# Julian-Wyatt/AnoDDPM

Hardware: AMD Instinct MI355X
Metric: reverse-diffusion images/sec @256x256 T=1000 simplex (higher is better)
Workload: dtype f32; 1 GPU; 256x256 simplex(8 oct) T=1000 base128 attn16,8 batch4/GPU (BASELINE config 2); per_gpu_batch=4, global_batch=4, T=1000, parallelism=batch-sharded x1 (no data-path collective), output_finite=True

## Files before the change

anoddpm_amd/csrc/attention.hip:

```cpp
#include "common.h"

namespace {

typedef float f32x4 __attribute__((ext_vector_type(4)));

constexpr int AT_LMAX = 1024;
constexpr int AT_WAVES = 8;
constexpr int AT_NT = AT_WAVES * 64;

template <int CHQ>
__global__ __launch_bounds__(AT_NT) void attention_kernel(const anoddpm_attention_args a)
{
    constexpr int CH = CHQ * 16;
    constexpr int QP = CH + 4;
    constexpr int TPW = CHQ >= AT_WAVES ? CHQ / AT_WAVES : 1;
    __shared__ __attribute__((aligned(16))) float lds[16 * (AT_LMAX + 4) + 16 * QP];
    const int L = a.L, SP = L + 4;
    float *S = lds, *Qs = lds + 16 * (AT_LMAX + 4);
    const int tid = threadIdx.x, lane = tid & 63, wave = tid >> 6;
    const int l16 = lane & 15, kq = lane >> 4;
    const int row0 = blockIdx.x * 16, hd = blockIdx.y, b = blockIdx.z;
    const int C3 = 3 * a.heads * CH;
    const float *__restrict__ qkv = a.qkv + (int64_t)b * L * C3 + hd * 3 * CH;
    const int nkt = L >> 4;

    for (int idx = tid; idx < 16 * (CH / 4); idx += AT_NT) {
        const int r = idx / (CH / 4), c4 = idx - r * (CH / 4);
        *reinterpret_cast<f32x4 *>(Qs + r * QP + c4 * 4) = *reinterpret_cast<const f32x4 *>(qkv + (int64_t)(row0 + r) * C3 + c4 * 4);
    }
    constexpr bool DB = CHQ < 32;
    f32x4 kb[DB ? 2 : 1][CHQ];
    auto load_k = [&](f32x4 (&dst)[CHQ], int jt) {
        const float *kp = qkv + (int64_t)(jt * 16 + l16) * C3 + CH + kq * 4;
#pragma unroll
        for (int g = 0; g < CHQ; ++g) dst[g] = *reinterpret_cast<const f32x4 *>(kp + g * 16);
    };
    auto score_tile = [&](const f32x4 (&kk)[CHQ], int jt) {
        f32x4 acc = {0.f, 0.f, 0.f, 0.f};
#pragma unroll
        for (int g = 0; g < CHQ; ++g) {
            const f32x4 qa = *reinterpret_cast<const f32x4 *>(Qs + l16 * QP + g * 16 + kq * 4);
#pragma unroll
            for (int e = 0; e < 4; ++e) acc = __builtin_amdgcn_mfma_f32_16x16x4f32(qa[e], kk[g][e], acc, 0, 0, 0);
        }
#pragma unroll
        for (int r = 0; r < 4; ++r) S[(kq * 4 + r) * SP + jt * 16 + l16] = acc[r] * a.scale;
    };
    if (wave < nkt) load_k(kb[0], wave);
    __syncthreads();
    if constexpr (DB) {
        for (int jt = wave; jt < nkt; jt += 2 * AT_WAVES) {
            if (jt + AT_WAVES < nkt) load_k(kb[1], jt + AT_WAVES);
            score_tile(kb[0], jt);
            if (jt + AT_WAVES < nkt) {
                if (jt + 2 * AT_WAVES < nkt) load_k(kb[0], jt + 2 * AT_WAVES);
                score_tile(kb[1], jt + AT_WAVES);
            }
        }
    } else {
        for (int jt = wave; jt < nkt; jt += AT_WAVES) {
            if (jt != wave) load_k(kb[0], jt);
            score_tile(kb[0], jt);
        }
    }
    const int ct0 = wave * TPW;
    const bool pv_active = ct0 < CHQ;
    float vb[2][TPW][4];
    auto load_v = [&](float (&dst)[TPW][4], int kg) {
        const float *vp = qkv + (int64_t)(kg * 16 + kq * 4) * C3 + 2 * CH + ct0 * 16 + l16;
#pragma unroll
        for (int t = 0; t < TPW; ++t)
#pragma unroll
            for (int e = 0; e < 4; ++e) dst[t][e] = vp[(int64_t)e * C3 + t * 16];
    };
    if (pv_active) load_v(vb[0], 0);
    __syncthreads();

    {
        constexpr int TPR = AT_NT / 16;
        const int r = tid / TPR, sub = tid % TPR;
        float *srow = S + r * SP;
        float m = -INFINITY;
        for (int j = sub; j < L; j += TPR) m = fmaxf(m, srow[j]);
#pragma unroll
        for (int o = TPR / 2; o >= 1; o >>= 1) m = fmaxf(m, __shfl_xor(m, o, TPR));
        float sum = 0.f;
        for (int j = sub; j < L; j += TPR) {
            const float e = __expf(srow[j] - m);
            srow[j] = e;
            sum += e;
        }
#pragma unroll
        for (int o = TPR / 2; o >= 1; o >>= 1) sum += __shfl_xor(sum, o, TPR);
        const float inv = 1.0f / sum;
        float *prow = a.probs ? a.probs + (((int64_t)b * a.heads + hd) * L + row0 + r) * L : nullptr;
        for (int j = sub; j < L; j += TPR) {
            const float p = srow[j] * inv;
            srow[j] = p;
            if (prow) prow[j] = p;
        }
    }
    __syncthreads();

    if (!pv_active) return;
    f32x4 oacc[TPW];
#pragma unroll
    for (int t = 0; t < TPW; ++t) oacc[t] = f32x4{0.f, 0.f, 0.f, 0.f};
    auto pv_group = [&](const float (&vv)[TPW][4], int kg) {
        const f32x4 pa = *reinterpret_cast<const f32x4 *>(S + l16 * SP + kg * 16 + kq * 4);
#pragma unroll
        for (int e = 0; e < 4; ++e)
#pragma unroll
            for (int t = 0; t < TPW; ++t) oacc[t] = __builtin_amdgcn_mfma_f32_16x16x4f32(pa[e], vv[t][e], oacc[t], 0, 0, 0);
    };
    for (int kg = 0; kg < nkt; kg += 2) {
        if (kg + 1 < nkt) load_v(vb[1], kg + 1);
        pv_group(vb[0], kg);
        if (kg + 1 < nkt) {
            if (kg + 2 < nkt) load_v(vb[0], kg + 2);
            pv_group(vb[1], kg + 1);
        }
    }
    float *__restrict__ O = a.out + ((int64_t)b * L + row0 + kq * 4) * (a.heads * CH) + hd * CH + ct0 * 16 + l16;
#pragma unroll
    for (int t = 0; t < TPW; ++t)
#pragma unroll
        for (int r = 0; r < 4; ++r) O[(int64_t)r * (a.heads * CH) + t * 16] = oacc[t][r];
}

}

extern "C" int anoddpm_attention(const anoddpm_attention_args *a, void *stream)
{
    ANODDPM_REQUIRE(a && a->qkv && a->out, "attention: null pointer");
    ANODDPM_REQUIRE(a->B >= 1 && a->heads >= 1 && a->B <= 65535 && a->heads <= 65535, "attention: bad batch / head count");
    ANODDPM_REQUIRE(a->L >= 16 && a->L % 16 == 0 && a->L <= AT_LMAX, "attention: L must be a multiple of 16 in [16, 1024]");
    ANODDPM_REQUIRE(a->ch >= 16 && a->ch <= 512 && (a->ch & (a->ch - 1)) == 0, "attention: head width must be a power of two in [16, 512]");
    ANODDPM_REQUIRE(((uintptr_t)a->qkv & 15) == 0, "attention: qkv must be 16-byte aligned");
    const dim3 grid((unsigned)(a->L / 16), (unsigned)a->heads, (unsigned)a->B);
    hipStream_t s = anoddpm::as_stream(stream);
    switch (a->ch / 16) {
        case 1: hipLaunchKernelGGL((attention_kernel<1>), grid, dim3(AT_NT), 0, s, *a); break;
        case 2: hipLaunchKernelGGL((attention_kernel<2>), grid, dim3(AT_NT), 0, s, *a); break;
        case 4: hipLaunchKernelGGL((attention_kernel<4>), grid, dim3(AT_NT), 0, s, *a); break;
        case 8: hipLaunchKernelGGL((attention_kernel<8>), grid, dim3(AT_NT), 0, s, *a); break;
        case 16: hipLaunchKernelGGL((attention_kernel<16>), grid, dim3(AT_NT), 0, s, *a); break;
        default: hipLaunchKernelGGL((attention_kernel<32>), grid, dim3(AT_NT), 0, s, *a); break;
    }
    return anoddpm::check_launch("attention");
}
```

anoddpm_amd/csrc/executor.hip:

```cpp
#include <stdarg.h>
#include <string.h>
#include <vector>
#include "common.h"

namespace anoddpm {

static thread_local char g_err[512] = "";
int g_debug[16] = {0};

void set_error(const char *fmt, ...)
{
    va_list ap;
    va_start(ap, fmt);
    vsnprintf(g_err, sizeof(g_err), fmt, ap);
    va_end(ap);
}

struct ProfState {
    bool on = false;
    std::vector<hipEvent_t> pool;
    std::vector<int> codes;
    std::vector<float> last_ms;
    std::vector<int> last_codes;
    size_t used = 0;
    double ms[ANODDPM_OP_MAX] = {0};
    int64_t launches[ANODDPM_OP_MAX] = {0};
};
static ProfState g_prof;

static int dispatch(const anoddpm_op &op, void *stream)
{
    switch (op.code) {
        case ANODDPM_OP_IGEMM: return anoddpm_igemm(static_cast<const anoddpm_igemm_args *>(op.args), stream);
        case ANODDPM_OP_GN_STATS: return anoddpm_gn_stats(static_cast<const anoddpm_gn_args *>(op.args), stream);
        case ANODDPM_OP_SOFTMAX: return anoddpm_softmax_rows(static_cast<const anoddpm_softmax_args *>(op.args), stream);
        case ANODDPM_OP_RESAMPLE: return anoddpm_resample2x(static_cast<const anoddpm_resample_args *>(op.args), stream);
        case ANODDPM_OP_LINEAR: return anoddpm_linear_small(static_cast<const anoddpm_linear_args *>(op.args), stream);
        case ANODDPM_OP_POSEMB: return anoddpm_posemb(static_cast<const anoddpm_posemb_args *>(op.args), stream);
        case ANODDPM_OP_STEM: return anoddpm_conv_stem(static_cast<const anoddpm_stem_args *>(op.args), stream);
        case ANODDPM_OP_LAYOUT: return anoddpm_nhwc_to_nchw(static_cast<const anoddpm_layout_args *>(op.args), stream);
        case ANODDPM_OP_CHAN_STATS: return anoddpm_chan_stats(static_cast<const anoddpm_chan_stats_args *>(op.args), stream);
        case ANODDPM_OP_HEAD: return anoddpm_conv_head(static_cast<const anoddpm_head_args *>(op.args), stream);
        case ANODDPM_OP_GN_FINALIZE: return anoddpm_gn_finalize(static_cast<const anoddpm_gn_finalize_args *>(op.args), stream);
        case ANODDPM_OP_WGRAD3: return anoddpm_conv3x3_wgrad(static_cast<const anoddpm_wgrad_args *>(op.args), stream);
        case ANODDPM_OP_WGRAD1: return anoddpm_wgrad_pointwise(static_cast<const anoddpm_wgrad1_args *>(op.args), stream);
        case ANODDPM_OP_GN_BWD: return anoddpm_gn_silu_backward(static_cast<const anoddpm_gn_bwd_args *>(op.args), stream);
        case ANODDPM_OP_PACK: return anoddpm_pack_weights(static_cast<const anoddpm_pack_args *>(op.args), stream);
        case ANODDPM_OP_SOFTMAX_BWD: return anoddpm_softmax_rows_backward(static_cast<const anoddpm_softmax_bwd_args *>(op.args), stream);
        case ANODDPM_OP_TRANSPOSE: return anoddpm_transpose_square(static_cast<const anoddpm_transpose_args *>(op.args), stream);
        case ANODDPM_OP_LINEAR_BWD: return anoddpm_linear_small_backward(static_cast<const anoddpm_linear_bwd_args *>(op.args), stream);
        case ANODDPM_OP_STEM_BWD: return anoddpm_conv_stem_backward(static_cast<const anoddpm_stem_bwd_args *>(op.args), stream);
        case ANODDPM_OP_HEAD_BWD: return anoddpm_conv_head_backward(static_cast<const anoddpm_head_bwd_args *>(op.args), stream);
        case ANODDPM_OP_COLSUM_FOLD: return anoddpm_colsum_fold(static_cast<const anoddpm_colsum_fold_args *>(op.args), stream);
        case ANODDPM_OP_ATTENTION: return anoddpm_attention(static_cast<const anoddpm_attention_args *>(op.args), stream);
        case ANODDPM_OP_PACK_BATCH: return anoddpm_pack_batch(static_cast<const anoddpm_pack_batch_args *>(op.args), stream);
        case ANODDPM_OP_DROPOUT: return anoddpm_dropout(static_cast<const anoddpm_dropout_args *>(op.args), stream);
        case ANODDPM_OP_LINEAR_BWD_BATCH: return anoddpm_linear_small_backward_batch(static_cast<const anoddpm_linear_bwd_batch_args *>(op.args), stream);
        default: set_error("run_ops: unknown op code %d", op.code); return ANODDPM_EINVAL;
    }
}

}

using namespace anoddpm;

extern "C" int anoddpm_internal_variant(int32_t key, int32_t value)
{
    if (key < 0 || key >= 16) return ANODDPM_EINVAL;
#ifndef ANODDPM_ABLATE
    if (!(key == 0 || key == 4 || key == 5 || key == 8 || key == 9)) {
        set_error("internal_variant: key %d selects a timing ablation; this library was built without ANODDPM_ABLATE", key);
        return ANODDPM_EINVAL;
    }
#endif
    g_debug[key] = value;
    return ANODDPM_OK;
}

extern "C" int anoddpm_ablate_build(void)
{
#ifdef ANODDPM_ABLATE
    return 1;
#else
    return 0;
#endif
}

extern "C" int anoddpm_abi_version(void) { return 24; }

extern "C" const char *anoddpm_last_error(void) { return g_err; }

extern "C" int anoddpm_device_count(void)
{
    int n = 0;
    if (hipGetDeviceCount(&n) != hipSuccess) { (void)hipGetLastError(); return 0; }
    return n;
}

extern "C" int anoddpm_run_ops(const anoddpm_op *ops, int32_t n, void *stream)
{
    ANODDPM_REQUIRE(ops || n == 0, "run_ops: null op list");
    for (int i = 0; i < n; ++i) {
        ANODDPM_REQUIRE(ops[i].args, "run_ops: op %d has null args", i);
        hipEvent_t e0 = nullptr, e1 = nullptr;
        const bool prof = g_prof.on && ops[i].code > 0 && ops[i].code < ANODDPM_OP_MAX;
        if (prof) {
            if (g_prof.used + 2 > g_prof.pool.size()) {
                hipEvent_t a, b;
                if (hipEventCreate(&a) != hipSuccess || hipEventCreate(&b) != hipSuccess) {
                    set_error("run_ops: hipEventCreate failed");
                    return ANODDPM_ELAUNCH;
                }
                g_prof.pool.push_back(a);
                g_prof.pool.push_back(b);
            }
            e0 = g_prof.pool[g_prof.used];
            e1 = g_prof.pool[g_prof.used + 1];
            g_prof.used += 2;
            const int icfg = ops[i].code == ANODDPM_OP_IGEMM ? static_cast<const anoddpm_igemm_args *>(ops[i].args)->cfg : 0;
            const bool w43 = ops[i].code == ANODDPM_OP_WGRAD3 && static_cast<const anoddpm_wgrad_args *>(ops[i].args)->algo == 1;
            g_prof.codes.push_back((icfg == 2 || icfg == 6) ? 12 : ((icfg == 3 || icfg == 7) ? 14 : (icfg == 5 ? 13 : (w43 ? 15 : ops[i].code))));
            (void)hipEventRecord(e0, as_stream(stream));
        }
        const int rc = dispatch(ops[i], stream);
        if (prof) (void)hipEventRecord(e1, as_stream(stream));
        if (rc != ANODDPM_OK) {
            char tmp[400];
            strncpy(tmp, g_err, sizeof(tmp) - 1);
            tmp[sizeof(tmp) - 1] = 0;
            set_error("op %d (code %d): %s", i, ops[i].code, tmp);
            return rc;
        }
    }
    return ANODDPM_OK;
}

extern "C" int anoddpm_prof_enable(int32_t enable)
{
    g_prof.on = enable != 0;
    if (enable) {
        g_prof.used = 0;
        g_prof.codes.clear();
        memset(g_prof.ms, 0, sizeof(g_prof.ms));
        memset(g_prof.launches, 0, sizeof(g_prof.launches));
    }
    return ANODDPM_OK;
}

extern "C" int anoddpm_prof_active(void) { return g_prof.on ? 1 : 0; }

extern "C" int anoddpm_prof_collect(double *ms_per_code, int64_t *launches_per_code)
{
    ANODDPM_REQUIRE(ms_per_code && launches_per_code, "prof_collect: null pointer");
    g_prof.last_ms.clear();
    g_prof.last_codes.clear();
    for (size_t i = 0; i < g_prof.codes.size(); ++i) {
        hipEvent_t e0 = g_prof.pool[2 * i], e1 = g_prof.pool[2 * i + 1];
        if (hipEventSynchronize(e1) != hipSuccess) { set_error("prof_collect: event sync failed"); return ANODDPM_ELAUNCH; }
        float ms = 0.f;
        if (hipEventElapsedTime(&ms, e0, e1) != hipSuccess) { set_error("prof_collect: elapsed failed"); return ANODDPM_ELAUNCH; }
        g_prof.ms[g_prof.codes[i]] += ms;
        g_prof.launches[g_prof.codes[i]] += 1;
        g_prof.last_ms.push_back(ms);
        g_prof.last_codes.push_back(g_prof.codes[i]);
    }
    g_prof.codes.clear();
    g_prof.used = 0;
    for (int c = 0; c < ANODDPM_OP_MAX; ++c) { ms_per_code[c] = g_prof.ms[c]; launches_per_code[c] = g_prof.launches[c]; }
    return ANODDPM_OK;
}

extern "C" int anoddpm_prof_list(int32_t *codes, float *ms, int32_t cap)
{
    const int n = (int)g_prof.last_ms.size();
    for (int i = 0; i < n && i < cap; ++i) {
        if (codes) codes[i] = g_prof.last_codes[i];
        if (ms) ms[i] = g_prof.last_ms[i];
    }
    return n;
}

extern "C" int anoddpm_struct_size(int32_t which)
{
    switch (which) {
        case 0: return (int)sizeof(anoddpm_simplex_args);
        case 1: return (int)sizeof(anoddpm_p_update_args);
        case 2: return (int)sizeof(anoddpm_igemm_args);
        case 3: return (int)sizeof(anoddpm_gn_args);
        case 4: return (int)sizeof(anoddpm_softmax_args);
        case 5: return (int)sizeof(anoddpm_resample_args);
        case 6: return (int)sizeof(anoddpm_linear_args);
        case 7: return (int)sizeof(anoddpm_posemb_args);
        case 8: return (int)sizeof(anoddpm_stem_args);
        case 9: return (int)sizeof(anoddpm_layout_args);
        case 10: return (int)sizeof(anoddpm_op);
        case 11: return (int)sizeof(anoddpm_adamw_args);
        case 12: return (int)sizeof(anoddpm_chan_stats_args);
        case 13: return (int)sizeof(anoddpm_gn_finalize_args);
        case 14: return (int)sizeof(anoddpm_head_args);
        case 15: return (int)sizeof(anoddpm_anomaly_args);
        case 16: return (int)sizeof(anoddpm_vlb_args);
        case 17: return (int)sizeof(anoddpm_wgrad_args);
        case 18: return (int)sizeof(anoddpm_gn_bwd_args);
        case 19: return (int)sizeof(anoddpm_wgrad1_args);
        case 20: return (int)sizeof(anoddpm_pack_args);
        case 21: return (int)sizeof(anoddpm_softmax_bwd_args);
        case 22: return (int)sizeof(anoddpm_transpose_args);
        case 23: return (int)sizeof(anoddpm_linear_bwd_args);
        case 24: return (int)sizeof(anoddpm_stem_bwd_args);
        case 25: return (int)sizeof(anoddpm_head_bwd_args);
        case 26: return (int)sizeof(anoddpm_colsum_fold_args);
        case 27: return (int)sizeof(anoddpm_mri_slice_args);
        case 28: return (int)sizeof(anoddpm_resize_args);
        case 29: return (int)sizeof(anoddpm_attention_args);
        case 30: return (int)sizeof(anoddpm_pack_batch_args);
        case 31: return (int)sizeof(anoddpm_linear_bwd_batch_args);
        case 32: return (int)sizeof(anoddpm_loss_args);
        case 33: return (int)sizeof(anoddpm_dropout_args);
        default: return -1;
    }
}
```

Before: 0.4478 images/s.

## Split attention PV output channels across extra workgroups to fill the GPU

The attention kernel can now split the head's output channels across several workgroups per 16-row block, with the slice count chosen so total workgroups reach about 256. Each slice recomputes the full QK^T scores and softmax, but only one writes the probabilities. The V prefetch depth also grows (up to 8 groups in flight when each wave owns few channel tiles). This trades redundant score and softmax work for more parallelism on small grids such as the 16x16 and 8x8 attention resolutions at batch 4.

```diff
diff --git a/anoddpm_amd/csrc/attention.hip b/anoddpm_amd/csrc/attention.hip
--- a/anoddpm_amd/csrc/attention.hip
+++ b/anoddpm_amd/csrc/attention.hip
@@ -7,19 +7,21 @@
 constexpr int AT_LMAX = 1024;
 constexpr int AT_WAVES = 8;
 constexpr int AT_NT = AT_WAVES * 64;
+constexpr int AT_MAX_SLICES = 16;
 
-template <int CHQ>
-__global__ __launch_bounds__(AT_NT) void attention_kernel(const anoddpm_attention_args a)
+template <int CHQ, int TPW>
+__global__ __launch_bounds__(AT_NT) void attention_kernel(const anoddpm_attention_args a, const int nslice)
 {
     constexpr int CH = CHQ * 16;
     constexpr int QP = CH + 4;
-    constexpr int TPW = CHQ >= AT_WAVES ? CHQ / AT_WAVES : 1;
+    constexpr int VR = TPW >= 4 ? 2 : 8 / TPW;
     __shared__ __attribute__((aligned(16))) float lds[16 * (AT_LMAX + 4) + 16 * QP];
     const int L = a.L, SP = L + 4;
     float *S = lds, *Qs = lds + 16 * (AT_LMAX + 4);
     const int tid = threadIdx.x, lane = tid & 63, wave = tid >> 6;
     const int l16 = lane & 15, kq = lane >> 4;
-    const int row0 = blockIdx.x * 16, hd = blockIdx.y, b = blockIdx.z;
+    const int rb = blockIdx.x / nslice, slice = blockIdx.x - rb * nslice;
+    const int row0 = rb * 16, hd = blockIdx.y, b = blockIdx.z;
     const int C3 = 3 * a.heads * CH;
     const float *__restrict__ qkv = a.qkv + (int64_t)b * L * C3 + hd * 3 * CH;
     const int nkt = L >> 4;
@@ -63,9 +65,10 @@
             score_tile(kb[0], jt);
         }
     }
-    const int ct0 = wave * TPW;
-    const bool pv_active = ct0 < CHQ;
-    float vb[2][TPW][4];
+    const int chs = CHQ / nslice;
+    const int ct0 = slice * chs + wave * TPW;
+    const bool pv_active = wave * TPW < chs;
+    float vb[VR][TPW][4];
     auto load_v = [&](float (&dst)[TPW][4], int kg) {
         const float *vp = qkv + (int64_t)(kg * 16 + kq * 4) * C3 + 2 * CH + ct0 * 16 + l16;
 #pragma unroll
@@ -73,7 +76,11 @@
 #pragma unroll
             for (int e = 0; e < 4; ++e) dst[t][e] = vp[(int64_t)e * C3 + t * 16];
     };
-    if (pv_active) load_v(vb[0], 0);
+    if (pv_active) {
+#pragma unroll
+        for (int i = 0; i < VR; ++i)
+            if (i < nkt) load_v(vb[i], i);
+    }
     __syncthreads();
 
     {
@@ -93,7 +100,7 @@
 #pragma unroll
         for (int o = TPR / 2; o >= 1; o >>= 1) sum += __shfl_xor(sum, o, TPR);
         const float inv = 1.0f / sum;
-        float *prow = a.probs ? a.probs + (((int64_t)b * a.heads + hd) * L + row0 + r) * L : nullptr;
+        float *prow = a.probs && slice == 0 ? a.probs + (((int64_t)b * a.heads + hd) * L + row0 + r) * L : nullptr;
         for (int j = sub; j < L; j += TPR) {
             const float p = srow[j] * inv;
             srow[j] = p;
@@ -113,12 +120,14 @@
 #pragma unroll
             for (int t = 0; t < TPW; ++t) oacc[t] = __builtin_amdgcn_mfma_f32_16x16x4f32(pa[e], vv[t][e], oacc[t], 0, 0, 0);
     };
-    for (int kg = 0; kg < nkt; kg += 2) {
-        if (kg + 1 < nkt) load_v(vb[1], kg + 1);
-        pv_group(vb[0], kg);
-        if (kg + 1 < nkt) {
-            if (kg + 2 < nkt) load_v(vb[0], kg + 2);
-            pv_group(vb[1], kg + 1);
+    for (int kg0 = 0; kg0 < nkt; kg0 += VR) {
+#pragma unroll
+        for (int i = 0; i < VR; ++i) {
+            const int kg = kg0 + i;
+            if (kg < nkt) {
+                pv_group(vb[i], kg);
+                if (kg + VR < nkt) load_v(vb[i], kg + VR);
+            }
         }
     }
     float *__restrict__ O = a.out + ((int64_t)b * L + row0 + kq * 4) * (a.heads * CH) + hd * CH + ct0 * 16 + l16;
@@ -126,6 +135,32 @@
     for (int t = 0; t < TPW; ++t)
 #pragma unroll
         for (int r = 0; r < 4; ++r) O[(int64_t)r * (a.heads * CH) + t * 16] = oacc[t][r];
+}
+
+static int attention_slices(int L, int chq, int heads, int B)
+{
+    const int forced = anoddpm::g_debug[10];
+    if (forced > 0) return forced;
+    const int64_t wg = (int64_t)(L / 16) * heads * B;
+    int ns = 1;
+    while (ns * 2 <= chq && ns * 2 <= AT_MAX_SLICES && wg * ns < 256) ns *= 2;
+    return ns;
+}
+
+template <int CHQ, int TPW>
+static void launch_tpw(const anoddpm_attention_args *a, int ns, hipStream_t s)
+{
+    const dim3 grid((unsigned)(a->L / 16 * ns), (unsigned)a->heads, (unsigned)a->B);
+    hipLaunchKernelGGL((attention_kernel<CHQ, TPW>), grid, dim3(AT_NT), 0, s, *a, ns);
+}
+
+template <int CHQ>
+static void launch_chq(const anoddpm_attention_args *a, int ns, hipStream_t s)
+{
+    const int tiles = CHQ / ns / AT_WAVES;
+    if constexpr (CHQ >= 4 * AT_WAVES) { if (tiles >= 4) return launch_tpw<CHQ, 4>(a, ns, s); }
+    if constexpr (CHQ >= 2 * AT_WAVES) { if (tiles >= 2) return launch_tpw<CHQ, 2>(a, ns, s); }
+    launch_tpw<CHQ, 1>(a, ns, s);
 }
 
 }
@@ -137,15 +172,18 @@
     ANODDPM_REQUIRE(a->L >= 16 && a->L % 16 == 0 && a->L <= AT_LMAX, "attention: L must be a multiple of 16 in [16, 1024]");
     ANODDPM_REQUIRE(a->ch >= 16 && a->ch <= 512 && (a->ch & (a->ch - 1)) == 0, "attention: head width must be a power of two in [16, 512]");
     ANODDPM_REQUIRE(((uintptr_t)a->qkv & 15) == 0, "attention: qkv must be 16-byte aligned");
-    const dim3 grid((unsigned)(a->L / 16), (unsigned)a->heads, (unsigned)a->B);
+    const int chq = a->ch / 16;
+    const int ns = attention_slices(a->L, chq, a->heads, a->B);
+    ANODDPM_REQUIRE(ns >= 1 && ns <= chq && ns <= AT_MAX_SLICES && (ns & (ns - 1)) == 0,
+                    "attention: slice count %d must be a power of two <= min(ch / 16, %d)", ns, AT_MAX_SLICES);
     hipStream_t s = anoddpm::as_stream(stream);
-    switch (a->ch / 16) {
-        case 1: hipLaunchKernelGGL((attention_kernel<1>), grid, dim3(AT_NT), 0, s, *a); break;
-        case 2: hipLaunchKernelGGL((attention_kernel<2>), grid, dim3(AT_NT), 0, s, *a); break;
-        case 4: hipLaunchKernelGGL((attention_kernel<4>), grid, dim3(AT_NT), 0, s, *a); break;
-        case 8: hipLaunchKernelGGL((attention_kernel<8>), grid, dim3(AT_NT), 0, s, *a); break;
-        case 16: hipLaunchKernelGGL((attention_kernel<16>), grid, dim3(AT_NT), 0, s, *a); break;
-        default: hipLaunchKernelGGL((attention_kernel<32>), grid, dim3(AT_NT), 0, s, *a); break;
+    switch (chq) {
+        case 1: launch_chq<1>(a, ns, s); break;
+        case 2: launch_chq<2>(a, ns, s); break;
+        case 4: launch_chq<4>(a, ns, s); break;
+        case 8: launch_chq<8>(a, ns, s); break;
+        case 16: launch_chq<16>(a, ns, s); break;
+        default: launch_chq<32>(a, ns, s); break;
     }
     return anoddpm::check_launch("attention");
 }
diff --git a/anoddpm_amd/csrc/executor.hip b/anoddpm_amd/csrc/executor.hip
--- a/anoddpm_amd/csrc/executor.hip
+++ b/anoddpm_amd/csrc/executor.hip
@@ -68,7 +68,7 @@
 {
     if (key < 0 || key >= 16) return ANODDPM_EINVAL;
 #ifndef ANODDPM_ABLATE
-    if (!(key == 0 || key == 4 || key == 5 || key == 8 || key == 9)) {
+    if (!(key == 0 || key == 4 || key == 5 || key == 8 || key == 9 || key == 10)) {
         set_error("internal_variant: key %d selects a timing ablation; this library was built without ANODDPM_ABLATE", key);
         return ANODDPM_EINVAL;
     }
```

After: 0.4490 images/s, median of 6. No clear change (+0.3%).
